# DrSleep/nas-segm-pytorch

Measured on AMD Instinct MI355X. Metric: images/sec (fwd+bwd+optimizer step) WACV arch0 2048x1024 bs=4/GPU, higher is better.
Workload: dtype f32

## Files before the change

include/nasseg.h:

```cpp
#ifndef NASSEG_H
#define NASSEG_H

#include <stdint.h>

#ifdef __cplusplus
extern "C" {
#endif

const char* nasseg_last_error(void);
int nasseg_abi_version(void);
int nasseg_device_count(void);

int nasseg_dw_pack_weight(const float* w, float* wt, int C, int K, int flip, void* stream);
int nasseg_dwconv(const float* x, const float* wt, float* y, const float* in_scale,
                  const float* in_shift, int in_act, const float* scale, const float* shift, int act,
                  int B, int H, int W, int C, int Ho, int Wo, int K, int stride, int pad, int dil,
                  int transposed, float* stats, void* stream);
int nasseg_dwconv_strip_ok(int K, int stride, int dil);
int64_t nasseg_dwconv_stats_blocks(int B, int C, int Ho, int Wo, int K, int stride, int dil);
int nasseg_dwconv_bwd_data_bn(const float* dy, const float* wt, float* g, const float* z,
                              const float* scale, const float* shift, const float* mean,
                              const float* invstd, int act, int B, int H, int W, int C, int Ho,
                              int Wo, int K, int stride, int pad, int dil, int transposed,
                              float* stats, void* stream);
int64_t nasseg_dwconv_bwd_data_bn_blocks(int B, int C, int Ho, int Wo, int K, int stride, int pad,
                                         int dil, int transposed);
int64_t nasseg_dwconv_bwd_bn_rows(int B, int C, int H, int W, int K, int stride, int pad, int dil);
int nasseg_dwconv_bwd_bn(const float* xz, const float* g, const float* z, const float* wt, int wt_flipped, float* ge,
                         float* dw, float* ws, const float* in_scale, const float* in_shift, const float* in_mean,
                         const float* in_invstd, int in_act, const float* bn_scale, const float* bn_shift,
                         const float* bn_mean, const float* bn_invstd, const float* bn_sums, int bn_train, int bn_act,
                         int B, int H, int W, int C, int Ho, int Wo, int K, int stride, int pad, int dil, float* stats,
                         void* stream);
int64_t nasseg_dwconv_wgrad_workspace(int B, int C, int Ho, int Wo, int K);
int nasseg_dwconv_wgrad(const float* x, const float* dy, float* dw, float* ws,
                        const float* in_scale, const float* in_shift, int in_act, int B, int H, int W,
                        int C, int Ho, int Wo, int K, int stride, int pad, int dil, void* stream);

int nasseg_dw_wgrad_lds(int v);

int64_t nasseg_sepconv_blocks(int B, int C, int Ho, int Wo, int N, int K, int stride, int dil);
int nasseg_sepconv_fwd(const float* x, const float* wdw, const float* wpw, float* zdw, float* y,
                       const float* in_scale, const float* in_shift, int in_act,
                       const float* out_scale, const float* out_shift, int out_act, int B, int H,
                       int W, int C, int Ho, int Wo, int N, int K, int stride, int pad, int dil,
                       float* stats, void* stream);

int64_t nasseg_irdw_rows(int B, int H, int W, int K, int C, int stride, int backward);
int64_t nasseg_irdw_stats_workspace(int K);
int nasseg_irdw_stats(const float* x, const float* w1, const float* in_scale, const float* in_shift, int in_act, int B,
                      int H, int W, int K, int C, float eps, float momentum, const float* gamma, const float* beta,
                      float* mean, float* invstd, float* scale, float* shift, float* running_mean, float* running_var,
                      int64_t* num_batches_tracked, float* ws, void* stream);
int nasseg_irdw_fwd(const float* x, const float* w1, const float* wdw, float* z2, const float* in_scale,
                    const float* in_shift, int in_act, const float* bn1_scale, const float* bn1_shift, int act1,
                    int B, int H, int W, int K, int C, int Ho, int Wo, int stride, float* stats, void* stream);
int nasseg_irdw_bwd(const float* x, const float* w1, const float* g, const float* z2, const float* wdw,
                    int wdw_flipped, float* ge, float* dw, float* ws, const float* in_scale, const float* in_shift,
                    int in_act, const float* bn1_scale, const float* bn1_shift, const float* bn1_mean,
                    const float* bn1_invstd, int act1, const float* bn2_scale, const float* bn2_shift,
                    const float* bn2_mean, const float* bn2_invstd, const float* bn2_sums, int bn2_train, int bn2_act,
                    int B, int H, int W, int K, int C, int Ho, int Wo, int stride, float* stats, void* stream);

int nasseg_conv_pack_weight(const float* w, float* wp, int N, int K, int kh, int kw, int mode,
                            void* stream);
int nasseg_pack_weights(int count, const float* const* w, float* const* wp, const int* dims,
                        void* stream);
int nasseg_conv_fwd_pack_mode(int K, int kh, int kw);
int nasseg_conv_fwd(const float* x, int ldx, const float* wp, float* y, int ldy,
                    const float* in_scale, const float* in_shift, int in_act,
                    const float* out_scale, const float* out_shift, int out_act, const float* res,
                    int ldres, int B, int Hs, int Ws, int K, int Ho, int Wo, int N, int kh, int kw,
                    int stride, int pad, int dil, int transposed, float* stats, void* stream);
int64_t nasseg_conv_fwd_stats_blocks(int B, int Ho, int Wo, int N, int K, int pointwise);
int64_t nasseg_conv_fwd_stats_rows(int B, int Ho, int Wo, int N, int K, int kh, int kw, int stride, int pad, int dil);
int64_t nasseg_conv_pw_min_pixels(int64_t v);
int nasseg_conv_pwn_mode(int v);
int nasseg_conv_deep_k(int v);
int nasseg_pool_strip(int v);
int64_t nasseg_conv_pointwise_kernel(int B, int Ho, int Wo, int N, int K, int pointwise);
int64_t nasseg_conv_fwd_lds3x3(int B, int Ho, int Wo, int N, int K, int kh, int kw, int stride, int pad, int dil,
                               int with_stats);
int nasseg_conv_bwd_data_bn(const float* dy, int lddy, const float* wp, float* g, int ldg,
                            const float* z, int ldz, const float* scale, const float* shift,
                            const float* mean, const float* invstd, int act, int B, int Hs, int Ws,
                            int K, int Ho, int Wo, int N, int kh, int kw, int stride, int pad,
                            int dil, float* stats, void* stream);
int nasseg_conv_wgrad_lds3x3(int B, int Hs, int Ws, int K, int Ho, int Wo, int N, int kh, int kw, int stride,
                             int pad, int dil);
int64_t nasseg_conv_wgrad_workspace(int B, int Ho, int Wo, int N, int K, int kh, int kw);
int nasseg_wgrad_finalize_many(int count, const float* const* partial, float* const* dw,
                               const int* dims, void* stream);
int nasseg_conv_wgrad_many(int count, const int64_t* desc, void* stream);
int nasseg_dwconv_wgrad_many(int count, const int64_t* desc, void* stream);

int nasseg_conv_wgrad_bn(const float* x, int ldx, const float* g, int ldg, const float* z, int ldz, float* dz,
                         int lddz, float* dw, float* ws, const float* in_scale, const float* in_shift, int in_act,
                         const float* bn_scale, const float* bn_shift, const float* bn_mean, const float* bn_invstd,
                         const float* bn_sums, int bn_train, int bn_act, int B, int H, int W, int K, int N, void* stream);
int nasseg_conv_wgrad_bn_flat(const float* x, int ldx, const float* g, int ldg, const float* z, int ldz, float* dw,
                              float* ws, const float* bn_scale, const float* bn_shift, const float* bn_mean,
                              const float* bn_invstd, const float* bn_sums, int bn_train, int bn_act, int B, int Hs,
                              int Ws, int K, int Ho, int Wo, int N, int kh, int kw, int stride, int pad, int dil,
                              void* stream);
int nasseg_dwconv_wgrad_bn(const float* x, const float* g, const float* z, float* dz, float* dw, float* ws,
                           const float* in_scale, const float* in_shift, int in_act, const float* bn_scale, const float* bn_shift,
                           const float* bn_mean, const float* bn_invstd, const float* bn_sums, int bn_train, int bn_act,
                           int B, int H, int W, int C, int Ho, int Wo, int K, int stride, int pad, int dil,
                           void* stream);
int64_t nasseg_conv_pw_bwd_slabs(int B, int H, int W, int K, int N);
int64_t nasseg_conv_pw_bwd_reads_z(int B, int H, int W, int K, int N);
int64_t nasseg_conv_pw_bwd_rz_min_pixels(int64_t v);
int nasseg_conv_pw_bwd_bn(const float* x, const float* g, const float* z, const float* wb, float* dx, float* dw,
                          float* ws, const float* in_scale, const float* in_shift, int in_act, int dx_act,
                          const float* bn_scale, const float* bn_shift, const float* bn_mean, const float* bn_invstd,
                          const float* bn_sums, int bn_train, int bn_act, int B, int H, int W, int K, int N,
                          const float* in_mean, const float* in_invstd, float* dx_stats, const float* dx_res,
                          void* stream);
int nasseg_conv_wgrad(const float* x, int ldx, const float* dy, int lddy, float* dw, float* ws,
                      const float* in_scale, const float* in_shift, int in_act, int B, int Hs,
                      int Ws, int K, int Ho, int Wo, int N, int kh, int kw, int stride, int pad,
                      int dil, void* stream);

int64_t nasseg_colred_workspace(int S, int64_t R, int C);
int nasseg_colred(int mode, const float* a, int64_t lda, const float* b, int64_t ldb,
                  const float* c, int64_t ldc, float* out, float* ws, int S, int64_t R, int C,
                  float mul, void* stream);
int nasseg_bn_stats(const float* x, int64_t ldx, int64_t M, int C, float eps, float momentum,
                    const float* gamma, const float* beta, float* mean, float* invstd,
                    float* scale, float* shift, float* running_mean, float* running_var,
                    int64_t* num_batches_tracked, float* ws, void* stream);
int nasseg_bn_finalize(float* partial, int nblk, int64_t M, int C, float eps, float momentum,
                       const float* gamma, const float* beta, float* mean, float* invstd,
                       float* scale, float* shift, float* running_mean, float* running_var,
                       int64_t* num_batches_tracked, void* stream);
int nasseg_bn_eval_params(int C, float eps, const float* gamma, const float* beta,
                          const float* running_mean, const float* running_var, float* mean,
                          float* invstd, float* scale, float* shift, void* stream);
int nasseg_bn_bwd_reduce(const float* dy, int64_t lddy, const float* x, int64_t ldx, int64_t M,
                         int C, const float* scale, const float* shift, const float* mean,
                         const float* invstd, int act, float* sums, float* ws, void* stream);
int nasseg_rows_sum(float* partial, int nblk, int cols, float* out, void* stream);
int nasseg_bn_bwd_apply(const float* dy, const float* x, const float* scale, const float* shift,
                        const float* mean, const float* invstd, const float* sums, int64_t M,
                        int C, int train, int act, float* dx, void* stream);
int64_t nasseg_colred_rows(int S, int64_t R, int C);
int64_t nasseg_bn_bwd_apply_rows_max_bytes(void);
int nasseg_bn_bwd_reduce_rows(const float* dy, int64_t lddy, const float* x, int64_t ldx, int64_t M, int C,
                              const float* scale, const float* shift, const float* mean, const float* invstd, int act,
                              float* rows, void* stream);
int nasseg_bn_bwd_apply_rows(const float* dy, const float* x, const float* scale, const float* shift, const float* mean,
                             const float* invstd, const float* rows, int nrows, float* sums_out, int64_t M, int C,
                             int train, int act, float* dx, void* stream);

int nasseg_affine_act(const float* x, const float* scale, const float* shift, const float* res,
                      float* y, int64_t n, int C, int act, void* stream);
int nasseg_axpby(const float* a, const float* b, const float* alpha, const float* beta, float* y,
                 int64_t n, int C, int act, void* stream);
int nasseg_add_act2(const float* xa, const float* sa, const float* ha, int act_a, const float* ca, const float* xb,
                    const float* sb, const float* hb, int act_b, const float* cb, float* y, int64_t n, int C,
                    void* stream);
// ... 296 lines not shown
```

nas-segm-pytorch_amd/csrc/conv_fwd.hip:

```cpp
#include "conv_args.h"

#include <atomic>
#include <cstdio>
#include <cstdlib>

#if NASSEG_FP32_ONLY
std::atomic<int> g_conv_deep_k{1};
#else
extern std::atomic<int> g_conv_deep_k;
#endif

namespace {

enum { KM_VEC = 0, KM_SCALAR = 1, KM_FLAT = 2 };

#ifndef NASSEG_CONV_KU
#define NASSEG_CONV_KU 1
#endif
#ifndef NASSEG_PW_MIN_PIXELS
#define NASSEG_PW_MIN_PIXELS -2
#endif
#ifndef NASSEG_LDS3X3_VALU_TAIL
#define NASSEG_LDS3X3_VALU_TAIL 1
#endif

template <bool VEC>
__device__ __forceinline__ float4 load4(const float* row, int k, int K) {
  if (VEC) {
    return lda4(row + (k < K ? k : 0));
  } else {
    float4 v;
    v.x = keep_if(row[k + 0 < K ? k + 0 : 0], k + 0 < K);
    v.y = keep_if(row[k + 1 < K ? k + 1 : 0], k + 1 < K);
    v.z = keep_if(row[k + 2 < K ? k + 2 : 0], k + 2 < K);
    v.w = keep_if(row[k + 3 < K ? k + 3 : 0], k + 3 < K);
    return v;
  }
}

#ifdef NASSEG_BF16
template <bool VEC>
__device__ __forceinline__ float4 load4(const bf16_t* row, int k, int K) {
  if (VEC) {
    return lda4(row + (k < K ? k : 0));
  } else {
    float4 v;
    v.x = keep_if(lda1(row + (k + 0 < K ? k + 0 : 0)), k + 0 < K);
    v.y = keep_if(lda1(row + (k + 1 < K ? k + 1 : 0)), k + 1 < K);
    v.z = keep_if(lda1(row + (k + 2 < K ? k + 2 : 0)), k + 2 < K);
    v.w = keep_if(lda1(row + (k + 3 < K ? k + 3 : 0)), k + 3 < K);
    return v;
  }
}
#endif

template <int MT, int NT, int KM, bool GATHER, bool PRO, bool VECN, bool EPI, int STATS, bool WS,
          int KU_ = NASSEG_CONV_KU>
__global__ __launch_bounds__(256) void conv_fwd_kernel(FwdArgs a) {
  constexpr bool kSums = STATS == 1 || STATS == 2;
  __shared__ float sred[(kSums && !WS) ? 4 : 1][2][(kSums && !WS) ? NT * 16 : 1];
  const int lane = threadIdx.x & 63;
  const int wave = threadIdx.x >> 6;
  const int j = lane & 15;
  const int kg = lane >> 4;
  const int Mtot = a.g.B * a.g.Ho * a.g.Wo;
  const int m_base = WS ? blockIdx.x * (16 * MT) : (blockIdx.x * 4 + wave) * (16 * MT);
  const bool active = m_base < Mtot;
  if ((!kSums || WS) && !active) return;
  const int n_base = WS ? (blockIdx.y * 4 + wave) * (16 * NT) : blockIdx.y * (16 * NT);
  if (WS && n_base >= a.N) return;

  int pm[MT], pb[MT], py[MT], px[MT];
#pragma unroll
  for (int mt = 0; mt < MT; ++mt) {
    const int m = m_base + mt * 16 + j;
    pm[mt] = m < Mtot ? m : Mtot - 1;
    if (GATHER) {
      px[mt] = pm[mt] % a.g.Wo;
      const int t = pm[mt] / a.g.Wo;
      py[mt] = t % a.g.Ho;
      pb[mt] = t / a.g.Ho;
    }
  }
  int wn[NT];
  bool wok[NT];
#pragma unroll
  for (int nt = 0; nt < NT; ++nt) {
    const int n = n_base + nt * 16 + j;
    wok[nt] = n < a.N;
    wn[nt] = wok[nt] ? n : a.N - 1;
  }

  f32x4 acc[MT][NT];
#pragma unroll
  for (int mt = 0; mt < MT; ++mt)
#pragma unroll
    for (int nt = 0; nt < NT; ++nt) acc[mt][nt] = (f32x4){0.f, 0.f, 0.f, 0.f};

  const int ntaps = a.g.kh * a.g.kw;
  constexpr int KU = (KM == KM_VEC) ? KU_ : 1;
  const ActSel pact = act_sel(a.in_act);
  const int Kq = (KM == KM_FLAT) ? ntaps * a.K : a.K;
  const int nk = (Kq + 15) >> 4;

  auto mma = [&](const float4* bv, const float4* av) {
#pragma unroll
// ... 522 lines not shown
    const int rounds = (th * tw + 63) / 64;
    const double kf = 0.25 * nt;
    const double alone = 14.0 + 8.0 * rounds * kf, shared = 14.0 + 2 * 10.5 * rounds * kf;
    const int64_t full = wgs / 512, rem = wgs % 512;
    return 5.0 + full * shared + (rem > 256 ? shared : (rem > 0 ? alone : 0.0)) +
           0.01 * (th + 2 * dil) * (tw + 2 * dil);
  };
  double bc = 0.9 * cost(best.th, best.tw);
  for (int tw = 8; tw <= 128 && tw <= Wo; ++tw) {
    for (int px = 64; px <= 256; px += 64) {
      const int th = px / tw < Ho ? px / tw : Ho;
      if (th < 1 || (th + 2 * dil) * (tw + 2 * dil) > kLdsMaxPatch) continue;
      const double c = cost(th, tw);
      if (c < bc) best = Lds3Tile{th, tw}, bc = c;
    }
  }
  return best;
}

template <int NT, bool VECN, bool VECK, int STATS = 0, int NV = 0, bool FLEX = false>
__global__ __launch_bounds__(256, 2) void conv3x3_lds_kernel(FwdArgs a) {
  static_assert(NV == 0 || (STATS == 0 && !VECN), "the vector-ALU channels come without statistics, stored one by one");
  extern __shared__ float tile[];
  __shared__ float sred3[STATS ? 4 : 1][2][STATS ? NT * 16 : 1];
  const int lane = threadIdx.x & 63;
  const int wave = threadIdx.x >> 6;
  const int j = lane & 15;
  const int kg = lane >> 4;
  const int dil = a.g.dil;
  const int th = FLEX ? a.th : kLdsTH, tw = FLEX ? a.tw : kLdsTW;
  const int TR = th + 2 * dil, TC = tw + 2 * dil;
  const int b = blockIdx.z;
  const int oy0 = blockIdx.y * th, ox0 = blockIdx.x * tw;
  const int iy0 = oy0 - a.g.pad, ix0 = ox0 - a.g.pad;
  const int H = a.g.Hs, W = a.g.Ws;

  int wn[NT];
  bool wok[NT];
#pragma unroll
  for (int nt = 0; nt < NT; ++nt) {
    const int n = nt * 16 + j;
    wok[nt] = n < a.N;
    wn[nt] = wok[nt] ? n : a.N - 1;
  }
  auto slot_pixel = [&](int mt, int& oy, int& ox) {
    if (!FLEX) {
      oy = oy0 + 2 * wave + (mt >> 1);
      ox = ox0 + (mt & 1) * 16 + j;
      return ((2 * wave + (mt >> 1)) * TC + (mt & 1) * 16 + j) * kLdsKS;
    }
    const int f = (4 * mt + wave) * 16 + j;
    const bool in_tile = f < th * tw;
    const int r = in_tile ? f / tw : 0;
    const int c = in_tile ? f - r * tw : 0;
    oy = in_tile ? oy0 + r : a.g.Ho;
    ox = ox0 + c;
    return (r * TC + c) * kLdsKS;
  };
  int toff[4];
#pragma unroll
  for (int mt = 0; mt < 4; ++mt) {
    int oy, ox;
    toff[mt] = slot_pixel(mt, oy, ox);
  }
  int nmt = 4;
  if (FLEX) {
    const int rem = th * tw - 16 * wave;
    nmt = rem <= 0 ? 0 : (rem + 63) / 64;
    nmt = nmt > 4 ? 4 : nmt;
  }

  f32x4 acc[4][NT];
#pragma unroll
  for (int mt = 0; mt < 4; ++mt)
#pragma unroll
    for (int nt = 0; nt < NT; ++nt) acc[mt][nt] = (f32x4){0.f, 0.f, 0.f, 0.f};
  float pv[4][NV ? NV : 1];
#pragma unroll
  for (int mt = 0; mt < 4; ++mt)
#pragma unroll
    for (int c = 0; c < (NV ? NV : 1); ++c) pv[mt][c] = 0.f;

  const act_t* xb = a.x + (int64_t)b * H * W * a.ldx;
  for (int kc0 = 0; kc0 < a.K; kc0 += kLdsKC) {
    if (kc0) __syncthreads();
    {
      const int total = TR * TC * (kLdsKC / 4);
      float4 rv[kLdsMaxIt];
#pragma unroll
      for (int it = 0; it < kLdsMaxIt; ++it) {
        int idx = threadIdx.x + 256 * it;
        idx = idx < total ? idx : total - 1;
        const int q = idx % (kLdsKC / 4);
        const int p = idx / (kLdsKC / 4);
        const int pc = p % TC, pr = p / TC;
        const int iy = iy0 + pr, ix = ix0 + pc;
        const int iyc = iy < 0 ? 0 : (iy >= H ? H - 1 : iy), ixc = ix < 0 ? 0 : (ix >= W ? W - 1 : ix);
        const int k = kc0 + q * 4;
        const act_t* src = xb + ((int64_t)iyc * W + ixc) * a.ldx;
        rv[it] = load4<VECK>(src, VECK ? (k < a.K ? k : 0) : k, a.K);
      }
#pragma unroll
      for (int it = 0; it < kLdsMaxIt; ++it) {
        const int idx = threadIdx.x + 256 * it;
        const int q = idx % (kLdsKC / 4);
        const int p = idx / (kLdsKC / 4);
        const int pc = p % TC, pr = p / TC;
        const int iy = iy0 + pr, ix = ix0 + pc;
        const bool ok = iy >= 0 && iy < H && ix >= 0 && ix < W;
        const int k = kc0 + q * 4;
        float4 v = rv[it];
        if (!VECK) {
          v.y = keep_if(v.y, k + 1 < a.K);
          v.z = keep_if(v.z, k + 2 < a.K);
          v.w = keep_if(v.w, k + 3 < a.K);
        }
        if (idx < total) *reinterpret_cast<float4*>(&tile[p * kLdsKS + q * 4]) = keep_if(v, ok && k < a.K);
      }
    }
    __syncthreads();
    const int nks = (a.K - kc0 >= kLdsKC) ? kLdsKC / 16 : (a.K - kc0 + 15) / 16;
    const int rem_last = a.K - kc0 - (nks - 1) * 16;
    const int ntail = rem_last <= 8 ? (rem_last + 3) / 4 : 0;
    const int nvec = ntail ? nks - 1 : nks;
    const int nsteps = 9 * nvec;
    auto step_of = [&](int it, int& tap, int& ks) {
      tap = nvec == 2 ? (it >> 1) : it;
      ks = nvec == 2 ? (it & 1) : 0;
    };
    auto load_w = [&](int it, float4 (&av)[NT], float4 (&xv)[NV ? NV : 1]) {
      int tap, ks;
      step_of(it, tap, ks);
      const int k = kc0 + ks * 16 + kg * 4;
#pragma unroll
      for (int nt = 0; nt < NT; ++nt) av[nt] = load4<VECK>(a.w + ((int64_t)tap * a.N + wn[nt]) * a.K, k, a.K);
#pragma unroll
      for (int c = 0; c < NV; ++c) xv[c] = load4<VECK>(a.w + ((int64_t)tap * a.N + NT * 16 + c) * a.K, k, a.K);
    };
    auto do_step = [&](int it, const float4 (&avr)[NT], const float4 (&xvr)[NV ? NV : 1]) {
      int tap, ks;
      step_of(it, tap, ks);
      const int ty = tap / 3, tx = tap - ty * 3;
      const int tsh = (ty * dil * TC + tx * dil) * kLdsKS;
      const int kl = ks * 16 + kg * 4;
      const int k = kc0 + kl;
      float4 bv[4], av[NT], xv[NV ? NV : 1];
#pragma unroll
      for (int mt = 0; mt < 4; ++mt)
        if (!FLEX || mt < nmt) bv[mt] = *reinterpret_cast<const float4*>(&tile[toff[mt] + tsh + kl]);
#pragma unroll
      for (int nt = 0; nt < NT; ++nt) {
        float4 v = avr[nt];
        if (!VECK) {
          v.y = keep_if(v.y, k + 1 < a.K);
          v.z = keep_if(v.z, k + 2 < a.K);
          v.w = keep_if(v.w, k + 3 < a.K);
        }
        av[nt] = keep_if(v, wok[nt] && k < a.K);
      }
#pragma unroll
      for (int c = 0; c < NV; ++c) xv[c] = keep_if(xvr[c], k < a.K);
#pragma unroll
      for (int mt = 0; mt < 4; ++mt) {
        if (FLEX && mt >= nmt) continue;
#pragma unroll
        for (int nt = 0; nt < NT; ++nt) {
          acc[mt][nt] = mfma16(av[nt].x, bv[mt].x, acc[mt][nt]);
          acc[mt][nt] = mfma16(av[nt].y, bv[mt].y, acc[mt][nt]);
          acc[mt][nt] = mfma16(av[nt].z, bv[mt].z, acc[mt][nt]);
          acc[mt][nt] = mfma16(av[nt].w, bv[mt].w, acc[mt][nt]);
        }
#pragma unroll
        for (int c = 0; c < NV; ++c) {
          pv[mt][c] = fmaf(bv[mt].x, xv[c].x, pv[mt][c]);
          pv[mt][c] = fmaf(bv[mt].y, xv[c].y, pv[mt][c]);
          pv[mt][c] = fmaf(bv[mt].z, xv[c].z, pv[mt][c]);
          pv[mt][c] = fmaf(bv[mt].w, xv[c].w, pv[mt][c]);
        }
      }
    };
    if (nsteps) {
      float4 avA[NT], avB[NT], xvA[NV ? NV : 1], xvB[NV ? NV : 1];
      load_w(0, avA, xvA);
      int it = 0;
#pragma unroll 1
      for (; it + 1 < nsteps; it += 2) {
        load_w(it + 1, avB, xvB);
        __builtin_amdgcn_sched_barrier(0);
        do_step(it, avA, xvA);
        __builtin_amdgcn_sched_barrier(0);
        load_w(it + 2 < nsteps ? it + 2 : it + 1, avA, xvA);
        __builtin_amdgcn_sched_barrier(0);
        do_step(it + 1, avB, xvB);
        __builtin_amdgcn_sched_barrier(0);
      }
      if (it < nsteps) do_step(it, avA, xvA);
    }
    for (int tap = 0; tap < (ntail ? 9 : 0); ++tap) {
      const int ty = tap / 3, tx = tap - ty * 3;
      const int tsh = (ty * dil * TC + tx * dil) * kLdsKS;
      for (int st = 0; st < ntail; ++st) {
        const int kls = nvec * 16 + st * 4 + kg;
        const int kk = kc0 + kls;
        float bs[4], as[NT];
#pragma unroll
        for (int mt = 0; mt < 4; ++mt) bs[mt] = (!FLEX || mt < nmt) ? tile[toff[mt] + tsh + kls] : 0.f;
#pragma unroll
        for (int nt = 0; nt < NT; ++nt)
          as[nt] = keep_if(a.w[((int64_t)tap * a.N + wn[nt]) * a.K + (kk < a.K ? kk : 0)], wok[nt] && kk < a.K);
#pragma unroll
        for (int mt = 0; mt < 4; ++mt) {
          if (FLEX && mt >= nmt) continue;
#pragma unroll
          for (int nt = 0; nt < NT; ++nt) acc[mt][nt] = mfma16(as[nt], bs[mt], acc[mt][nt]);
        }
#pragma unroll
        for (int c = 0; c < NV; ++c) {
          const float wv = keep_if(a.w[((int64_t)tap * a.N + NT * 16 + c) * a.K + (kk < a.K ? kk : 0)], kk < a.K);
#pragma unroll
          for (int mt = 0; mt < 4; ++mt) pv[mt][c] = fmaf(bs[mt], wv, pv[mt][c]);
        }
      }
    }
  }
  if constexpr (NV > 0) {
#pragma unroll
    for (int mt = 0; mt < 4; ++mt)
#pragma unroll
      for (int c = 0; c < NV; ++c) {
        float v = pv[mt][c];
        v += __shfl_xor(v, 16, 64);
        v += __shfl_xor(v, 32, 64);
        pv[mt][c] = v;
      }
  }

  if constexpr (STATS == 1) {
#pragma unroll
    for (int nt = 0; nt < NT; ++nt) {
      float sx[4] = {0.f, 0.f, 0.f, 0.f}, sq[4] = {0.f, 0.f, 0.f, 0.f};
#pragma unroll
      for (int mt = 0; mt < 4; ++mt) {
        int oy, ox;
        slot_pixel(mt, oy, ox);
        const bool pok = oy < a.g.Ho && ox < a.g.Wo;
        const f32x4 c = acc[mt][nt];
#pragma unroll
        for (int r = 0; r < 4; ++r) {
          const float v = keep_if(c[r], pok);
          sx[r] += v;
          sq[r] = fmaf(v, v, sq[r]);
        }
      }
#pragma unroll
      for (int r = 0; r < 4; ++r) {
        sx[r] = row16_allsum(sx[r]);
        sq[r] = row16_allsum(sq[r]);
      }
      if (j == 0) {
#pragma unroll
        for (int r = 0; r < 4; ++r) {
          sred3[wave][0][nt * 16 + kg * 4 + r] = sx[r];
          sred3[wave][1][nt * 16 + kg * 4 + r] = sq[r];
        }
      }
    }
    __syncthreads();
    const int64_t row = ((int64_t)blockIdx.z * gridDim.y + blockIdx.y) * gridDim.x + blockIdx.x;
    for (int t = threadIdx.x; t < NT * 16; t += 256) {
      if (t < a.N) {
        float* po = a.stats + row * 2 * a.N + t;
        po[0] = (sred3[0][0][t] + sred3[1][0][t]) + (sred3[2][0][t] + sred3[3][0][t]);
        po[a.N] = (sred3[0][1][t] + sred3[1][1][t]) + (sred3[2][1][t] + sred3[3][1][t]);
      }
    }
  }
// ... 196 lines not shown
    }                                                                                             \
  } while (0)
#define GO(KM_, G_, P_, V_)                                   \
  do {                                                        \
    if constexpr (MT == 1 && KM_ == KM_VEC) {                 \
      if (deep) GO_(KM_, G_, P_, V_, 4);                      \
      else GO_(KM_, G_, P_, V_, NASSEG_CONV_KU);              \
    } else {                                                  \
      GO_(KM_, G_, P_, V_, NASSEG_CONV_KU);                   \
    }                                                         \
  } while (0)
  if (md.km == KM_FLAT) {
    if constexpr (NT <= 4 && !WS) {
      if (md.vecn) GO(KM_FLAT, true, false, true);
      else GO(KM_FLAT, true, false, false);
    } else {
      return nasseg_fail(NASSEG_ERR_UNSUPPORTED, "conv_fwd: flat path supports N <= 64");
    }
  } else if (!md.vecn) {
    if constexpr (NT <= 2 && !WS) {
      if (md.km == KM_VEC) GO(KM_VEC, true, false, false);
      else GO(KM_SCALAR, true, false, false);
    } else {
      return nasseg_fail(NASSEG_ERR_UNSUPPORTED, "conv_fwd: N %% 4 != 0 needs N <= 32");
    }
  } else if (md.km == KM_SCALAR) {
    GO(KM_SCALAR, true, false, true);
  } else if (md.gather) {
    GO(KM_VEC, true, false, true);
  } else if (md.pro) {
    GO(KM_VEC, false, true, true);
  } else {
    GO(KM_VEC, false, false, true);
  }
#undef GO
#undef GO_
  NASSEG_LAUNCH_CHECK("conv_fwd_kernel");
  return NASSEG_OK;
}

inline int pick_mt(int64_t Mtot, int tiles) {
  if (tiles > 4) return Mtot >= 16 * 4 * 1536 ? 4 : (Mtot >= 16 * 2 * 1536 ? 2 : 1);
  return Mtot >= 64 * 4 * 1536 ? 4 : (Mtot >= 64 * 2 * 1536 ? 2 : 1);
}
template <int NT, bool WS = false>
int launch_small(const FwdArgs& a, const Mode& md, hipStream_t s) {
  const int mt = pick_mt((int64_t)a.g.B * a.g.Ho * a.g.Wo, WS ? 5 : NT);
  if (mt == 4) return launch_one<4, NT, WS>(a, md, s);
  if (mt == 2) return launch_one<2, NT, WS>(a, md, s);
  return launch_one<1, NT, WS>(a, md, s);
}

template <int NT, int MT>
int launch_pw_nt(const FwdArgs& a, const PwFwdPlan& p, int stats, hipStream_t s) {
  const dim3 grid(p.grid), block(256);
  switch (stats) {
    case 0: hipLaunchKernelGGL((conv_pw_kernel<NT, MT, 0>), grid, block, p.lds, s, a); break;
    case 1: hipLaunchKernelGGL((conv_pw_kernel<NT, MT, 1>), grid, block, p.lds, s, a); break;
    case 2: hipLaunchKernelGGL((conv_pw_kernel<NT, MT, 2>), grid, block, p.lds, s, a); break;
    default: hipLaunchKernelGGL((conv_pw_kernel<NT, MT, 3>), grid, block, p.lds, s, a); break;
  }
  NASSEG_LAUNCH_CHECK("conv_pw_kernel");
  return NASSEG_OK;
}
int launch_pw(const FwdArgs& a, const PwFwdPlan& p, int stats, hipStream_t s) {
  switch (p.nt) {
    case 1: return launch_pw_nt<1, 2>(a, p, stats, s);
    case 2: return launch_pw_nt<2, 2>(a, p, stats, s);
    case 3: return launch_pw_nt<3, 2>(a, p, stats, s);
    case 4: return launch_pw_nt<4, 2>(a, p, stats, s);
    case 6: return launch_pw_nt<6, 2>(a, p, stats, s);
    case 9: return launch_pw_nt<9, 1>(a, p, stats, s);
    case 12: return launch_pw_nt<12, 1>(a, p, stats, s);
    default: return launch_pw_nt<14, 1>(a, p, stats, s);
  }
}

inline bool conv_small_ws(int64_t Mtot, int N, int K) {
  return g_conv_deep_k.load() != 0 && Mtot <= kDeepKMaxPixels && (N & 3) == 0 && (K & 3) == 0 && K >= 8 &&
         (int64_t)N * K <= 196608;
}

inline bool lds3x3_geometry(int B, int Ho, int Wo, int N, int K, int kh, int kw, int stride, int pad, int dil) {
  return kh == 3 && kw == 3 && stride == 1 && dil >= 1 && dil <= kLdsMaxDil && K * 9 > 64 && cdiv(N, 16) <= 4 &&
         Wo >= kLdsTW && Ho >= kLdsTH && B <= 65535 && pad >= 0 && pad <= 2 * dil;
}

inline int fwd_pack_mode(int K, int kh, int kw) { return (kh * kw > 1 && kh * kw * K <= 64) ? 2 : 0; }

int conv_dispatch(FwdArgs& a, int stats_mode, hipStream_t s) {
  const int K = a.K, N = a.N;
  const ConvGeom& g = a.g;
  NASSEG_REQUIRE(g.B > 0 && g.Hs > 0 && g.Ws > 0 && g.Ho > 0 && g.Wo > 0, "conv_fwd: bad geometry");
  NASSEG_REQUIRE(K > 0 && N > 0 && a.ldx >= K && a.ldy >= N, "conv_fwd: bad channels K=%d N=%d", K, N);
  NASSEG_REQUIRE((int64_t)g.B * g.Hs * g.Ws < 2147483647LL && (int64_t)g.B * g.Ho * g.Wo < 2147483647LL,
                 "conv_fwd: too many pixels");
  Mode md;
  md.km = (((K & 3) == 0) && ((a.ldx & 3) == 0)) ? KM_VEC : KM_SCALAR;
  md.pro = a.in_scale || a.in_shift || a.in_act;
  md.gather = !(g.kh == 1 && g.kw == 1 && g.stride == 1 && g.pad == 0 && g.Hs == g.Ho && g.Ws == g.Wo);
  md.vecn = ((N & 3) == 0) && ((a.ldy & 3) == 0) && (!a.res || (a.ldres & 3) == 0);
  md.epi = a.out_scale || a.out_shift || a.out_act || a.res;
  md.stats = stats_mode;
  NASSEG_REQUIRE(!md.stats || (md.vecn && !md.epi),
                 "conv_fwd: statistics need N %% 4 == 0 and no output epilogue");
  NASSEG_REQUIRE(md.stats < 2 || !md.pro, "conv_bwd_data_bn: no input prologue on this path");
  if (!g.transposed && fwd_pack_mode(K, g.kh, g.kw) == 2) md.km = KM_FLAT;
  NASSEG_REQUIRE(!md.pro || (md.km == KM_VEC && !md.gather && md.vecn),
                 "conv_fwd: the input prologue needs a pointwise conv with K %% 4 == 0, N %% 4 == 0");
  NASSEG_REQUIRE(a.y || (md.stats == 1 && !md.gather && md.km != KM_FLAT),
                 "conv_fwd: y == NULL needs statistics rows and a pointwise conv");
  const int tiles = cdiv(N, 16);
  if (!md.gather && md.km != KM_FLAT) {
    const PwnPlan pn = nasseg_internal_pwn_plan((int64_t)g.B * g.Ho * g.Wo, N, K, stats_mode >= 2 ? 2 : 1);
    if (pn.ok) {
      const bool aligned = md.km == KM_VEC && md.vecn && (stats_mode < 2 || (a.ldbz & 3) == 0);
      NASSEG_REQUIRE(aligned || (md.stats != 1 && md.stats != 2),
                     "conv_fwd: the pointwise statistics path needs channel strides that are multiples of 4");
      if (aligned) return NASSEG_INTERNAL(pwn_launch)(a, pn, md.stats, s);
    }
    NASSEG_REQUIRE(a.y, "conv_fwd: y == NULL (statistics only) is served by the N-split pointwise kernel alone");
    const PwFwdPlan pw = pw_fwd_plan((int64_t)g.B * g.Ho * g.Wo, N, K, stats_mode >= 2 ? 2 : 1);
    if (pw.ok) {
      const bool aligned = md.km == KM_VEC && md.vecn;
      NASSEG_REQUIRE(aligned || (md.stats != 1 && md.stats != 2),
                     "conv_fwd: the pointwise statistics path needs channel strides that are multiples of 4");
      if (aligned) return launch_pw(a, pw, md.stats, s);
    }
  }
  if (!g.transposed && lds3x3_geometry(g.B, g.Ho, g.Wo, N, K, g.kh, g.kw, g.stride, g.pad, g.dil) && md.km != KM_FLAT &&
      !md.pro && (md.stats == 0 || (md.stats == 1 && md.vecn))) {
    const bool veck = md.km == KM_VEC;
    if (NASSEG_LDS3X3_VALU_TAIL && veck && md.stats == 0 && N > 16 && N <= 21) {
      switch (N - 16) {
        case 1: return launch_lds3x3_nv<1, 1>(a, s);
        case 2: return launch_lds3x3_nv<1, 2>(a, s);
        case 3: return launch_lds3x3_nv<1, 3>(a, s);
        case 4: return launch_lds3x3_nv<1, 4>(a, s);
        default: return launch_lds3x3_nv<1, 5>(a, s);
      }
    }
    if (tiles <= 1) return launch_lds3x3<1>(a, md.vecn, veck, md.stats == 1, s);
    if (tiles == 2) return launch_lds3x3<2>(a, md.vecn, veck, md.stats == 1, s);
    return launch_lds3x3<4>(a, md.vecn, veck, md.stats == 1, s);
  }
  const bool rows_asked = md.stats == 1 || md.stats == 2;
  if (conv_small_ws((int64_t)g.B * g.Ho * g.Wo, N, K) && (rows_asked || K * g.kh * g.kw <= 1024)) {
    if (md.km == KM_VEC && md.vecn) return launch_one<1, 1, true>(a, md, s);
    NASSEG_REQUIRE(md.stats != 1 && md.stats != 2,
                   "conv_fwd: statistics on a small map need channel strides that are multiples of 4");
  }
  if (tiles <= 1) return launch_small<1>(a, md, s);
  if (tiles == 2) return launch_small<2>(a, md, s);
  if (tiles == 3) return launch_small<3>(a, md, s);
  if (tiles == 4) return launch_small<4>(a, md, s);
  if (tiles <= 8) return launch_small<2, true>(a, md, s);
  if (tiles <= 12) return launch_small<3, true>(a, md, s);
  return launch_small<4, true>(a, md, s);
}

}

extern "C" {

#if NASSEG_FP32_ONLY
int nasseg_conv_pack_weight(const float* w, float* wp, int N, int K, int kh, int kw, int mode,
                            void* stream) {
  NASSEG_REQUIRE(N > 0 && K > 0 && kh > 0 && kw > 0, "conv_pack_weight: bad shape");
  NASSEG_REQUIRE(mode >= 0 && mode <= 2, "conv_pack_weight: bad mode %d", mode);
  const int64_t total = (int64_t)N * K * kh * kw;
  hipLaunchKernelGGL(conv_pack_kernel, dim3((unsigned)cdiv64(total, 256)), dim3(256), 0,
                     (hipStream_t)stream, w, wp, N, K, kh * kw, mode);
  NASSEG_LAUNCH_CHECK("conv_pack_weight");
  return NASSEG_OK;
}
#endif

#if NASSEG_FP32_ONLY
int nasseg_pack_weights(int count, const float* const* w, float* const* wp, const int* dims,
                        void* stream) {
  NASSEG_REQUIRE(count >= 0 && (count == 0 || (w && wp && dims)), "pack_weights: bad arguments");
  for (int base = 0; base < count; base += kPackMax) {
    const int n = count - base < kPackMax ? count - base : kPackMax;
    PackTable t;
    int64_t most = 0;
    for (int i = 0; i < n; ++i) {
      const int* d = dims + 7 * (base + i);
      NASSEG_REQUIRE(d[0] > 0 && d[1] > 0 && d[2] > 0 && d[3] > 0 && d[4] >= 0 && d[4] <= 5,
                     "pack_weights: bad descriptor %d", base + i);
      NASSEG_REQUIRE(d[4] < 3 || d[4] == 5 || d[1] == 1, "pack_weights: depthwise weights have K = 1");
      NASSEG_REQUIRE(w[base + i] && wp[base + i], "pack_weights: null tensor %d", base + i);
      t.d[i].w = w[base + i];
      t.d[i].wp = wp[base + i];
      t.d[i].N = d[0];
      t.d[i].K = d[1];
      t.d[i].ntaps = d[2] * d[3];
      t.d[i].kind = d[4];
      t.d[i].Ksrc = d[5] > 0 ? d[5] : d[1];
      t.d[i].koff = d[5] > 0 ? d[6] : 0;
      NASSEG_REQUIRE(t.d[i].koff >= 0 && t.d[i].koff + d[1] <= t.d[i].Ksrc, "pack_weights: bad slice %d",
                     base + i);
      const int64_t total = (int64_t)d[0] * d[1] * d[2] * d[3];
      NASSEG_REQUIRE(total < 2147483647LL, "pack_weights: tensor %d too large", base + i);
      if (total > most) most = total;
    }
    int64_t gx = cdiv64(most, 256);
    if (gx > 256) gx = 256;
    hipLaunchKernelGGL(pack_multi_kernel, dim3((unsigned)gx, n), dim3(256), 0, (hipStream_t)stream, t);
    NASSEG_LAUNCH_CHECK("pack_weights");
  }
  return NASSEG_OK;
}
#endif

#if NASSEG_FP32_ONLY
int64_t nasseg_conv_pw_min_pixels(int64_t v) {
  return v == -1 ? g_pw_min_pixels.load() : g_pw_min_pixels.exchange(v < 0 ? -2 : v);
}
int nasseg_conv_deep_k(int v) {
  if (v < 0) return g_conv_deep_k.load();
  return g_conv_deep_k.exchange(v ? 1 : 0);
}
#endif

#if NASSEG_FP32_ONLY
int64_t nasseg_conv_fwd_stats_blocks(int B, int Ho, int Wo, int N, int K, int pointwise) {
  const int64_t Mtot = (int64_t)B * Ho * Wo;
  const int tiles = cdiv(N, 16);
  if (pointwise) {
    const PwnPlan pn = nasseg_internal_pwn_plan(Mtot, N, K, pointwise);
    if (pn.ok) return pointwise == 1 ? 2 * pn.grid : pn.grid;
    const PwFwdPlan pw = pw_fwd_plan(Mtot, N, K, pointwise);
    if (pw.ok) return pw.grid;
  }
  if (conv_small_ws(Mtot, N, K)) return cdiv64(Mtot, 16);
  return cdiv64(Mtot, (tiles > 4 ? 16 : 64) * pick_mt(Mtot, tiles));
}
#endif

#if NASSEG_FP32_ONLY
int64_t nasseg_conv_fwd_stats_rows(int B, int Ho, int Wo, int N, int K, int kh, int kw, int stride, int pad, int dil) {
  const int pointwise = (kh == 1 && kw == 1 && stride == 1 && pad == 0) ? 1 : 0;
  if (!pointwise && (N & 3) == 0 && lds3x3_geometry(B, Ho, Wo, N, K, kh, kw, stride, pad, dil))
  {
    const Lds3Tile t = cdiv(N, 16) > 2 ? lds3x3_tile(B, Ho, Wo, dil, 4) : Lds3Tile{kLdsTH, kLdsTW};
    return (int64_t)cdiv(Wo, t.tw) * cdiv(Ho, t.th) * B;
  }
  return nasseg_conv_fwd_stats_blocks(B, Ho, Wo, N, K, pointwise);
}
#endif

#if NASSEG_FP32_ONLY
int64_t nasseg_conv_pointwise_kernel(int B, int Ho, int Wo, int N, int K, int pointwise) {
  const int64_t Mtot = (int64_t)B * Ho * Wo;
  if (pointwise) {
    if (nasseg_internal_pwn_plan(Mtot, N, K, pointwise).ok) return 2;
    if (pw_fwd_plan(Mtot, N, K, pointwise).ok) return 1;
  }
  return 0;
}
#endif

#if NASSEG_FP32_ONLY
int64_t nasseg_conv_fwd_lds3x3(int B, int Ho, int Wo, int N, int K, int kh, int kw, int stride, int pad, int dil,
                               int with_stats) {
  return lds3x3_geometry(B, Ho, Wo, N, K, kh, kw, stride, pad, dil) && fwd_pack_mode(K, kh, kw) != 2 &&
                 (!with_stats || (N & 3) == 0)
             ? 1
             : 0;
}
#endif

#if NASSEG_FP32_ONLY
int nasseg_conv_fwd_pack_mode(int K, int kh, int kw) { return fwd_pack_mode(K, kh, kw); }
#endif

int NASSEG_FN(conv_fwd)(const act_t* x, int ldx, const float* wp, act_t* y, int ldy,
                    const float* in_scale, const float* in_shift, int in_act,
                    const float* out_scale, const float* out_shift, int out_act, const act_t* res,
                    int ldres, int B, int Hs, int Ws, int K, int Ho, int Wo, int N, int kh, int kw,
                    int stride, int pad, int dil, int transposed, float* stats, void* stream) {
  FwdArgs a = {};
  a.x = x; a.ldx = ldx; a.w = wp; a.y = y; a.ldy = ldy;
  a.in_scale = in_scale; a.in_shift = in_shift; a.in_act = in_act;
  a.out_scale = out_scale; a.out_shift = out_shift; a.out_act = out_act;
  a.res = res; a.ldres = ldres; a.stats = stats; a.K = K; a.N = N;
  a.g.B = B; a.g.Hs = Hs; a.g.Ws = Ws; a.g.Ho = Ho; a.g.Wo = Wo;
  a.g.kh = kh; a.g.kw = kw; a.g.stride = stride; a.g.pad = pad; a.g.dil = dil;
  a.g.transposed = transposed;
  return conv_dispatch(a, stats ? 1 : 0, (hipStream_t)stream);
}

int NASSEG_FN(conv_bwd_data_bn)(const act_t* dy, int lddy, const float* wp, act_t* g, int ldg,
                            const act_t* z, int ldz, const float* scale, const float* shift,
                            const float* mean, const float* invstd, int act, int B, int Hs, int Ws,
                            int K, int Ho, int Wo, int N, int kh, int kw, int stride, int pad,
                            int dil, float* stats, void* stream) {
  NASSEG_REQUIRE(z && (!stats || (scale && shift && mean && invstd)), "conv_bwd_data_bn: null argument");
  NASSEG_REQUIRE((ldz & 3) == 0 && ldz >= N, "conv_bwd_data_bn: bad ldz");
  FwdArgs a = {};
  a.x = dy; a.ldx = lddy; a.w = wp; a.y = g; a.ldy = ldg;
  a.stats = stats; a.K = K; a.N = N;
  a.bz = z; a.ldbz = ldz; a.b_scale = scale; a.b_shift = shift; a.b_mean = mean;
  a.b_invstd = invstd; a.b_act = act;
  a.g.B = B; a.g.Hs = Hs; a.g.Ws = Ws; a.g.Ho = Ho; a.g.Wo = Wo;
// ... 7 lines not shown
```

Before: 305.0.

## Prefetch next LDS input chunk during MFMA steps in 3x3 conv kernel

The LDS 3x3 conv forward kernel now precomputes per-thread source pixel offsets and in-bounds masks once, then issues the global loads for the next K-chunk of the input patch while the current chunk's MFMA steps run. The weight-load double buffer is also restructured so both buffers are preloaded and refilled after each step. This is meant to hide global-load latency behind compute, at the cost of extra live registers, which may lower occupancy. A runtime toggle to disable the LDS 3x3 path is also added.

```diff
diff --git a/include/nasseg.h b/include/nasseg.h
--- a/include/nasseg.h
+++ b/include/nasseg.h
@@ -77,6 +77,7 @@
 int64_t nasseg_conv_pw_min_pixels(int64_t v);
 int nasseg_conv_pwn_mode(int v);
 int nasseg_conv_deep_k(int v);
+int nasseg_conv_lds3x3(int v);
 int nasseg_pool_strip(int v);
 int64_t nasseg_conv_pointwise_kernel(int B, int Ho, int Wo, int N, int K, int pointwise);
 int64_t nasseg_conv_fwd_lds3x3(int B, int Ho, int Wo, int N, int K, int kh, int kw, int stride, int pad, int dil,
diff --git a/nas-segm-pytorch_amd/csrc/conv_fwd.hip b/nas-segm-pytorch_amd/csrc/conv_fwd.hip
--- a/nas-segm-pytorch_amd/csrc/conv_fwd.hip
+++ b/nas-segm-pytorch_amd/csrc/conv_fwd.hip
@@ -6,8 +6,10 @@
 
 #if NASSEG_FP32_ONLY
 std::atomic<int> g_conv_deep_k{1};
+std::atomic<int> g_conv_lds3x3{1};
 #else
 extern std::atomic<int> g_conv_deep_k;
+extern std::atomic<int> g_conv_lds3x3;
 #endif
 
 namespace {
@@ -22,6 +24,9 @@
 #endif
 #ifndef NASSEG_LDS3X3_VALU_TAIL
 #define NASSEG_LDS3X3_VALU_TAIL 1
+#endif
+#ifndef NASSEG_LDS3X3_PREFETCH
+#define NASSEG_LDS3X3_PREFETCH 1
 #endif
 
 template <bool VEC>
@@ -710,42 +715,53 @@
     for (int c = 0; c < (NV ? NV : 1); ++c) pv[mt][c] = 0.f;
 
   const act_t* xb = a.x + (int64_t)b * H * W * a.ldx;
+  const int total = TR * TC * (kLdsKC / 4);
+  int psrc[kLdsMaxIt];
+  unsigned pin = 0;
+#pragma unroll
+  for (int it = 0; it < kLdsMaxIt; ++it) {
+    int idx = threadIdx.x + 256 * it;
+    idx = idx < total ? idx : total - 1;
+    const int p = idx / (kLdsKC / 4);
+    const int pc = p % TC, pr = p / TC;
+    const int iy = iy0 + pr, ix = ix0 + pc;
+    const int iyc = iy < 0 ? 0 : (iy >= H ? H - 1 : iy), ixc = ix < 0 ? 0 : (ix >= W ? W - 1 : ix);
+    psrc[it] = iyc * W + ixc;
+    pin |= (iy >= 0 && iy < H && ix >= 0 && ix < W) ? (1u << it) : 0u;
+  }
+  float4 rv[kLdsMaxIt];
+  auto issue_patch = [&](int kc0) {
+#pragma unroll
+    for (int it = 0; it < kLdsMaxIt; ++it) {
+      if (256 * it >= total) continue;
+      int idx = threadIdx.x + 256 * it;
+      idx = idx < total ? idx : total - 1;
+      const int k = kc0 + (idx % (kLdsKC / 4)) * 4;
+      rv[it] = load4<VECK>(xb + (int64_t)psrc[it] * a.ldx, VECK ? (k < a.K ? k : 0) : k, a.K);
+    }
+  };
+  auto place_patch = [&](int kc0) {
+#pragma unroll
+    for (int it = 0; it < kLdsMaxIt; ++it) {
+      if (256 * it >= total) continue;
+      const int idx = threadIdx.x + 256 * it;
+      const int q = idx % (kLdsKC / 4);
+      const int p = idx / (kLdsKC / 4);
+      const int k = kc0 + q * 4;
+      float4 v = rv[it];
+      if (!VECK) {
+        v.y = keep_if(v.y, k + 1 < a.K);
+        v.z = keep_if(v.z, k + 2 < a.K);
+        v.w = keep_if(v.w, k + 3 < a.K);
+      }
+      if (idx < total) *reinterpret_cast<float4*>(&tile[p * kLdsKS + q * 4]) = keep_if(v, ((pin >> it) & 1u) && k < a.K);
+    }
+  };
+  issue_patch(0);
   for (int kc0 = 0; kc0 < a.K; kc0 += kLdsKC) {
     if (kc0) __syncthreads();
-    {
-      const int total = TR * TC * (kLdsKC / 4);
-      float4 rv[kLdsMaxIt];
-#pragma unroll
-      for (int it = 0; it < kLdsMaxIt; ++it) {
-        int idx = threadIdx.x + 256 * it;
-        idx = idx < total ? idx : total - 1;
-        const int q = idx % (kLdsKC / 4);
-        const int p = idx / (kLdsKC / 4);
-        const int pc = p % TC, pr = p / TC;
-        const int iy = iy0 + pr, ix = ix0 + pc;
-        const int iyc = iy < 0 ? 0 : (iy >= H ? H - 1 : iy), ixc = ix < 0 ? 0 : (ix >= W ? W - 1 : ix);
-        const int k = kc0 + q * 4;
-        const act_t* src = xb + ((int64_t)iyc * W + ixc) * a.ldx;
-        rv[it] = load4<VECK>(src, VECK ? (k < a.K ? k : 0) : k, a.K);
-      }
-#pragma unroll
-      for (int it = 0; it < kLdsMaxIt; ++it) {
-        const int idx = threadIdx.x + 256 * it;
-        const int q = idx % (kLdsKC / 4);
-        const int p = idx / (kLdsKC / 4);
-        const int pc = p % TC, pr = p / TC;
-        const int iy = iy0 + pr, ix = ix0 + pc;
-        const bool ok = iy >= 0 && iy < H && ix >= 0 && ix < W;
-        const int k = kc0 + q * 4;
-        float4 v = rv[it];
-        if (!VECK) {
-          v.y = keep_if(v.y, k + 1 < a.K);
-          v.z = keep_if(v.z, k + 2 < a.K);
-          v.w = keep_if(v.w, k + 3 < a.K);
-        }
-        if (idx < total) *reinterpret_cast<float4*>(&tile[p * kLdsKS + q * 4]) = keep_if(v, ok && k < a.K);
-      }
-    }
+    if (!NASSEG_LDS3X3_PREFETCH && kc0) issue_patch(kc0);
+    place_patch(kc0);
     __syncthreads();
     const int nks = (a.K - kc0 >= kLdsKC) ? kLdsKC / 16 : (a.K - kc0 + 15) / 16;
     const int rem_last = a.K - kc0 - (nks - 1) * 16;
@@ -807,19 +823,25 @@
         }
       }
     };
+    float4 avA[NT], avB[NT], xvA[NV ? NV : 1], xvB[NV ? NV : 1];
     if (nsteps) {
-      float4 avA[NT], avB[NT], xvA[NV ? NV : 1], xvB[NV ? NV : 1];
       load_w(0, avA, xvA);
+      load_w(1, avB, xvB);
+    }
+    if (NASSEG_LDS3X3_PREFETCH && kc0 + kLdsKC < a.K) issue_patch(kc0 + kLdsKC);
+    if (nsteps) {
+      const int last = nsteps - 1;
       int it = 0;
+      __builtin_amdgcn_sched_barrier(0);
 #pragma unroll 1
       for (; it + 1 < nsteps; it += 2) {
-        load_w(it + 1, avB, xvB);
-        __builtin_amdgcn_sched_barrier(0);
         do_step(it, avA, xvA);
         __builtin_amdgcn_sched_barrier(0);
-        load_w(it + 2 < nsteps ? it + 2 : it + 1, avA, xvA);
+        load_w(it + 2 < last ? it + 2 : last, avA, xvA);
         __builtin_amdgcn_sched_barrier(0);
         do_step(it + 1, avB, xvB);
+        __builtin_amdgcn_sched_barrier(0);
+        load_w(it + 3 < last ? it + 3 : last, avB, xvB);
         __builtin_amdgcn_sched_barrier(0);
       }
       if (it < nsteps) do_step(it, avA, xvA);
@@ -1182,8 +1204,8 @@
 }
 
 inline bool lds3x3_geometry(int B, int Ho, int Wo, int N, int K, int kh, int kw, int stride, int pad, int dil) {
-  return kh == 3 && kw == 3 && stride == 1 && dil >= 1 && dil <= kLdsMaxDil && K * 9 > 64 && cdiv(N, 16) <= 4 &&
-         Wo >= kLdsTW && Ho >= kLdsTH && B <= 65535 && pad >= 0 && pad <= 2 * dil;
+  return g_conv_lds3x3.load() != 0 && kh == 3 && kw == 3 && stride == 1 && dil >= 1 && dil <= kLdsMaxDil && K * 9 > 64 &&
+         cdiv(N, 16) <= 4 && Wo >= kLdsTW && Ho >= kLdsTH && B <= 65535 && pad >= 0 && pad <= 2 * dil;
 }
 
 inline int fwd_pack_mode(int K, int kh, int kw) { return (kh * kw > 1 && kh * kw * K <= 64) ? 2 : 0; }
@@ -1321,6 +1343,10 @@
   if (v < 0) return g_conv_deep_k.load();
   return g_conv_deep_k.exchange(v ? 1 : 0);
 }
+int nasseg_conv_lds3x3(int v) {
+  if (v < 0) return g_conv_lds3x3.load();
+  return g_conv_lds3x3.exchange(v ? 1 : 0);
+}
 #endif
 
 #if NASSEG_FP32_ONLY
```

After: 304.4, median of 2. Within noise of the previous version (-0.2%).
